# ethanhe42/epipolar-transformers

Hardware: NVIDIA B200
Metric: epipolar_fusion_forward_views_per_sec (higher is better)
Workload: dtype f32

## Files before the change

### epipolar_transformers_b200/csrc/epi_kernels.cuh

```cuda
#pragma once
#include <cuda_bf16.h>

#include "epi_common.cuh"

namespace epi {

struct FusionArgs {
    const float *feat_ref;  int64_t ref_stride[4];
    const float *src_nhwc;
    const __nv_bfloat16 *src_hi, *src_lo;
    const __nv_bfloat16 *ref_hi, *ref_lo;
    const uint16_t *order;
    const float *P_ref, *P_src;
    const float *locs_in;
    float *out;             int64_t out_stride[4];
    __nv_bfloat16 *out_hi, *out_lo;
    float *attn, *corr_pos, *locs_out;
    int N, C;
    float softmax_scale;
    int add_ref;
    int *tile_counter;
    const PairGeom *pair_geom;
    int *err_flag;
    uint8_t *plan_cache;
    int plan_records;
    const uint32_t *pair_epoch;
    GeomCfg geom;
};

struct BwdArgs {
    const float *feat_ref;  int64_t ref_stride[4];
    const float *src_nhwc;
    const float *P_ref, *P_src, *locs_in;
    const float *attn;
    const float *grad_out;  int64_t gout_stride[4];
    const float *grad_attn;
    float *grad_ref;        int64_t gref_stride[4];
    float *dsrc_nhwc;
    int N, C;
    float softmax_scale;
    int grad_keys, grad_vals;
    GeomCfg geom;
};
cudaError_t launch_fusion_bwd(const BwdArgs &a, cudaStream_t st);

struct ZArgs {
    const float *x;         int64_t x_stride[4];
    const float *ref;       int64_t ref_stride[4];
    float *y;               int64_t y_stride[4];
    const float *Wf, *bf;
    int N, C, HW, W;
    int z_residual, add_ref;
};

struct ZGemmArgs {
    const __nv_bfloat16 *x_hi, *x_lo;
    const __nv_bfloat16 *w_hi, *w_lo;
    const float *Wf, *bf;
    const float *ref;       int64_t ref_stride[4];
    float *y;               int64_t y_stride[4];
    int N, C, HW, W, Npad;
    int z_residual, add_ref;
};
bool zgemm_supported(int C);
cudaError_t launch_zgemm(const ZGemmArgs &z, cudaStream_t st);

cudaError_t launch_fusion_warp(const FusionArgs &a, cudaStream_t st);
cudaError_t launch_fusion_tile(const FusionArgs &a, cudaStream_t st);
cudaError_t launch_fusion_pipe(const FusionArgs &a, cudaStream_t st);
bool fusion_pipe_shape_ok(int C, int H, int W, int K, bool has_locs_in);
size_t fusion_pipe_plan_record_bytes();
int fusion_pipe_plan_records(int N, int H, int W);
bool fusion_tile_supported(const FusionArgs &a);
bool fusion_tile_shape_ok(int C, int H, int W, int K, bool has_locs_in);
cudaError_t launch_sector_order(const float *P_ref, const float *P_src, uint16_t *order, int N, const GeomCfg &gc, cudaStream_t st);
cudaError_t launch_split_planes(const float *src, const int64_t stride[4], __nv_bfloat16 *hi, __nv_bfloat16 *lo, int N, int C,
                                int H, int W, int *zero_me, cudaStream_t st);

cudaError_t launch_stage(const float *ref, const int64_t ref_stride[4], const float *src, const int64_t src_stride[4],
                         __nv_bfloat16 *planes, const float *P_ref, const float *P_src, PairGeom *pair_geom, uint16_t *order,
                         float *order_key, const float *Wf, __nv_bfloat16 *w_planes, int w_add_identity, int *zero_words, int N, int C,
                         int H, int W, const GeomCfg &gc, cudaStream_t st);

cudaError_t launch_nchw_to_nhwc(const float *src, const int64_t stride[4], float *dst, int N, int C, int H, int W, cudaStream_t st);
cudaError_t launch_z_epilogue(const ZArgs &z, cudaStream_t st);
cudaError_t launch_unstage(const float *pm, const float *ref, const int64_t ref_stride[4], float *out, const int64_t out_stride[4],
                           int N, int C, int H, int W, cudaStream_t st);
cudaError_t launch_fold_z_bn(const float *zw, const float *zb, const float *g, const float *b, const float *mean,
                             const float *var, float eps, int C, float *wf, float *bf, cudaStream_t st);
cudaError_t launch_peaks(const float *heat, float *locs, float *scores, int B, int J, int H, int W, float radius, float downsample,
                         float threshold, int int_div, cudaStream_t st);
cudaError_t launch_sample_locs(const float *P_ref, const float *P_src, float *locs, int N, const GeomCfg &gc, cudaStream_t st);

}
```

### epipolar_transformers_b200/csrc/epi_stage.cu

```cuda
#include <cuda_bf16.h>

#include "epi_kernels.cuh"

namespace epi {

namespace stg {
constexpr int NT = 256;
constexpr int NBIN = 4096;
constexpr int SMALL = 32;
constexpr int TC = 64, TPX = 64, TPITCH = 65;

__device__ __forceinline__ float pseudo_angle(float u, float v) {
    const float p = __fdividef(v, fabsf(u) + fabsf(v) + 1e-30f);
    return u >= 0.f ? p : (v >= 0.f ? 2.f - p : -2.f - p);
}
__device__ __forceinline__ float angle_key(float px, float py, float ex, float ey, float cdx, float cdy, bool parallel, float lo, float inv_span) {
    float u;
    if (parallel) u = (px * (-cdy) + py * cdx - lo) * inv_span;
    else {
        const float dx = px - ex, dy = py - ey;
        u = (pseudo_angle(dx * cdx + dy * cdy, dy * cdx - dx * cdy) - lo) * inv_span;
    }
    u = fminf(fmaxf(u, 0.f), 0.99999f);
    if (!(u == u)) u = 0.f;
    return u;
}
}

#ifdef EPI_PIPE_TIMERS
__device__ unsigned long long g_stage_timers[16];
#define ST(slot) do { __syncthreads(); if (t == 0 && blockIdx.x == 0) { const long long t_ = clock64(); g_stage_timers[slot] = (unsigned long long)(t_ - st_prev); st_prev = t_; } } while (0)
extern "C" void epi_stage_timers_read(unsigned long long *out16) { cudaMemcpyFromSymbol(out16, g_stage_timers, sizeof(unsigned long long) * 16); }
#else
#define ST(slot) do { } while (0)
#endif

struct StageArgs {
    const float *ref, *src;
    int64_t ref_stride[4], src_stride[4];
    __nv_bfloat16 *planes;
    const float *P_ref, *P_src;
    PairGeom *pair_geom;
    uint16_t *order;
    int *zero_words;
    float *order_key;
    const float *Wf;
    int w_add_identity;
    __nv_bfloat16 *w_planes;
    int N, C, H, W;
    int do_ref, do_src, do_order;
    int persist;
    GeomCfg gc;
};

__global__ void __launch_bounds__(stg::NT, 5) epi_stage_kernel(const StageArgs s) {
    using namespace stg;
    extern __shared__ __align__(16) uint8_t dyn[];
    float (*tile)[TPITCH] = reinterpret_cast<float (*)[TPITCH]>(dyn);
    const int t = threadIdx.x;
    const int H = s.H, W = s.W, HW = H * W, C = s.C;
    const int nord = s.do_order ? s.N : 0;
    pdl_launch_dependents();
    pdl_wait();
    if (blockIdx.x == 0 && t == 0 && s.zero_words) { s.zero_words[0] = 0; s.zero_words[1] = 0; }

    if ((int)blockIdx.x < nord) {
        int *hist = reinterpret_cast<int *>(dyn);
        uint16_t *lst = reinterpret_cast<uint16_t *>(dyn + NBIN * 4);
        __shared__ float s_e[8];
        __shared__ int s_warp[NT / 32];
        __shared__ int s_big[64], s_nbig;
#ifdef EPI_PIPE_TIMERS
        long long st_prev = clock64();
#endif
        const int n = blockIdx.x;
        float my_key = 0.f;
        if (t < 32) {
            if (t < 12) my_key = s.P_ref[12 * n + t];
            else if (t < 24) my_key = s.P_src[12 * n + t - 12];
            else if (t == 24) my_key = (float)H;
            else if (t == 25) my_key = (float)W;
            else if (t == 26) my_key = s.gc.ds;
            else if (t == 27) my_key = s.gc.r;
            else if (t == 28) my_key = 1.f;
            else if (t == 29) my_key = (float)(s.gc.K + 1024 * s.gc.correct + 2048 * s.gc.align);
            else if (t == 30) my_key = s.gc.eps;
            if (s.order_key) {
                const bool same = t == 31 || __float_as_uint(s.order_key[32 * n + t]) == __float_as_uint(my_key);
                if (__all_sync(0xffffffffu, same)) s_e[7] = 1.f; else s_e[7] = 0.f;
            } else s_e[7] = 0.f;
        }
        __syncthreads();
        if (s_e[7] != 0.f) return;
        if (t == 0) {
            const float *P1 = s.P_ref + 12 * n, *P2 = s.P_src + 12 * n;
            PairGeom g;
            pair_geom_from_krt(P1, P2, g);
            s.pair_geom[n] = g;
            double b[9], t2[3];
            for (int r = 0; r < 3; r++) { for (int q = 0; q < 3; q++) b[r * 3 + q] = (double)P2[r * 4 + q]; t2[r] = (double)P2[r * 4 + 3]; }
            const double c00 = b[4] * b[8] - b[5] * b[7], c01 = b[5] * b[6] - b[3] * b[8], c02 = b[3] * b[7] - b[4] * b[6];
            const double id = 1.0 / (b[0] * c00 + b[1] * c01 + b[2] * c02);
            double bi[9];
            bi[0] = c00 * id; bi[1] = (b[2] * b[7] - b[1] * b[8]) * id; bi[2] = (b[1] * b[5] - b[2] * b[4]) * id;
            bi[3] = c01 * id; bi[4] = (b[0] * b[8] - b[2] * b[6]) * id; bi[5] = (b[2] * b[3] - b[0] * b[5]) * id;
            bi[6] = c02 * id; bi[7] = (b[1] * b[6] - b[0] * b[7]) * id; bi[8] = (b[0] * b[4] - b[1] * b[3]) * id;
            double cs[3], e[3];
            for (int r = 0; r < 3; r++) cs[r] = -(bi[r * 3] * t2[0] + bi[r * 3 + 1] * t2[1] + bi[r * 3 + 2] * t2[2]);
            for (int r = 0; r < 3; r++) e[r] = (double)P1[r * 4] * cs[0] + (double)P1[r * 4 + 1] * cs[1] + (double)P1[r * 4 + 2] * cs[2] + (double)P1[r * 4 + 3];
            const double cx = 0.5 * ((double)s.gc.xmin + s.gc.xmax), cy = 0.5 * ((double)s.gc.ymin + s.gc.ymax);
            const double nrm = fabs(e[0]) + fabs(e[1]) + 1e-300;
            const float cxs[4] = {s.gc.xmin, s.gc.xmax, s.gc.xmin, s.gc.xmax}, cys[4] = {s.gc.ymin, s.gc.ymin, s.gc.ymax, s.gc.ymax};
            float lo = 1e30f, hi = -1e30f, exf = 0.f, eyf = 0.f, cdx, cdy, par;
            if (!(fabs(e[2]) > 1e-9 * nrm)) {
                cdx = (float)(e[0] / nrm); cdy = (float)(e[1] / nrm); par = 1.f;
                for (int q = 0; q < 4; q++) { const float v = cxs[q] * (-cdy) + cys[q] * cdx; lo = fminf(lo, v); hi = fmaxf(hi, v); }
            } else {
                const double ex = e[0] / e[2], ey = e[1] / e[2];
                const double dn = sqrt((cx - ex) * (cx - ex) + (cy - ey) * (cy - ey)) + 1e-300;
                exf = (float)ex; eyf = (float)ey; cdx = (float)((cx - ex) / dn); cdy = (float)((cy - ey) / dn); par = 0.f;
                const bool inside = ex >= s.gc.xmin && ex <= s.gc.xmax && ey >= s.gc.ymin && ey <= s.gc.ymax;
                if (inside) { lo = -2.f; hi = 2.f; }
                else
                    for (int q = 0; q < 4; q++) {
                        const float dx = cxs[q] - exf, dy = cys[q] - eyf;
                        const float v = pseudo_angle(dx * cdx + dy * cdy, dy * cdx - dx * cdy);
                        lo = fminf(lo, v); hi = fmaxf(hi, v);
                    }
            }
            if (!(hi > lo)) { lo = 0.f; hi = 1.f; }
            s_e[0] = exf; s_e[1] = eyf; s_e[2] = cdx; s_e[3] = cdy; s_e[4] = par; s_e[5] = lo; s_e[6] = 1.f / ((hi - lo) * 1.0001f + 1e-20f);
            s_nbig = 0;
        }
        for (int b = t; b < NBIN; b += NT) hist[b] = 0;
        __syncthreads();
        ST(0);
        const float ex = s_e[0], ey = s_e[1], cdx = s_e[2], cdy = s_e[3], klo = s_e[5], kinv = s_e[6];
        const bool parallel = s_e[4] != 0.f;
        constexpr int MAXPT = 64;
        const int npt = (HW - t + NT - 1) / NT;
        const bool keep = npt <= MAXPT;
        uint16_t bins[MAXPT];
        auto bin_of = [&](int x, int y) -> int {
            return (int)(angle_key(pix2coord(x, s.gc.ds, s.gc.r), pix2coord(y, s.gc.ds, s.gc.r), ex, ey, cdx, cdy, parallel, klo, kinv) * (float)NBIN);
        };
        const int sx = NT % W, sy = NT / W;
        if (keep) {
            int x = t % W, y = t / W;
#pragma unroll 4
            for (int m = 0; m < MAXPT; m++) {
                if (m < npt) {
                    const int b = bin_of(x, y);
                    bins[m] = (uint16_t)b;
                    atomicAdd(&hist[b], 1);
                    x += sx; y += sy;
                    if (x >= W) { x -= W; y++; }
                }
            }
        } else {
            int x = t % W, y = t / W;
            for (int m = 0; m < npt; m++) {
                atomicAdd(&hist[bin_of(x, y)], 1);
                x += sx; y += sy;
                if (x >= W) { x -= W; y++; }
            }
        }
        __syncthreads();
        ST(1);
        constexpr int PER = NBIN / NT;
        int loc[PER], sum = 0;
#pragma unroll
        for (int q = 0; q < PER; q++) { loc[q] = hist[t * PER + q]; sum += loc[q]; }
        int incl = sum;
#pragma unroll
        for (int o = 1; o < 32; o <<= 1) { const int v = __shfl_up_sync(0xffffffffu, incl, o); if ((t & 31) >= o) incl += v; }
        if ((t & 31) == 31) s_warp[t >> 5] = incl;
        __syncthreads();
        int base = incl - sum;
        for (int w = 0; w < (t >> 5); w++) base += s_warp[w];
        const int start0 = base;
        __syncthreads();
#pragma unroll
        for (int q = 0; q < PER; q++) { hist[t * PER + q] = base; base += loc[q]; }
        __syncthreads();
        ST(2);
        if (keep) {
#pragma unroll 4
            for (int m = 0; m < MAXPT; m++)
                if (m < npt) lst[atomicAdd(&hist[bins[m]], 1)] = (uint16_t)(t + NT * m);
        } else {
            int x = t % W, y = t / W;
            for (int m = 0; m < npt; m++) {
                lst[atomicAdd(&hist[bin_of(x, y)], 1)] = (uint16_t)(t + NT * m);
                x += sx; y += sy;
                if (x >= W) { x -= W; y++; }
            }
        }
        __syncthreads();
        ST(3);
        uint16_t *ord = s.order + (size_t)n * HW;
        {
            int st0 = start0;
#pragma unroll
            for (int q = 0; q < PER; q++) {
                const int len = loc[q];
                bool coop = false;
                if (len > (keep ? SMALL : 4 * SMALL)) {
                    const int slot = atomicAdd(&s_nbig, 1);
                    if (slot < 64) { s_big[slot] = t * PER + q; coop = true; }
                }
                if (!coop) {
                    for (int e = 1; e < len; e++) {
                        const uint16_t xv = lst[st0 + e];
                        int p = e;
                        while (p > 0 && lst[st0 + p - 1] > xv) { lst[st0 + p] = lst[st0 + p - 1]; p--; }
                        lst[st0 + p] = xv;
                    }
                }
                st0 += len;
            }
        }
        __syncthreads();
        ST(4);
        const int nbig = s_nbig < 64 ? s_nbig : 64;
        for (int i = t; i < HW; i += NT) ord[i] = lst[i];
        for (int bb = 0; bb < nbig; bb++) {
            const int b = s_big[bb];
            const int end = hist[b], beg = b == 0 ? 0 : hist[b - 1];
            __syncthreads();
            for (int e = beg + t; e < end; e += NT) {
                const uint16_t xv = lst[e];
                int r = 0;
                for (int f = beg; f < end; f++) r += lst[f] < xv;
                ord[beg + r] = xv;
            }
        }
        if (s.order_key) {
            __syncthreads();
            if (t < 31) s.order_key[32 * n + t] = my_key;
            else if (t == 31) reinterpret_cast<uint32_t *>(s.order_key)[32 * n + 31] += 1u;
        }
        return;
    }

    const int tiles_p = (HW + TPX - 1) / TPX, tiles_c = (C + TC - 1) / TC;
    const int per_map = tiles_p * tiles_c * s.N;
    int lin = (int)blockIdx.x - nord;
    const int wblocks = (s.Wf && s.w_planes) ? (C * C / 8 + NT - 1) / NT : 0;
    const int wlin = s.persist ? lin : lin - 2 * per_map;
    if (wlin >= 0 && wlin < wblocks) {
        const size_t e0 = ((size_t)wlin * NT + t) * 8, tot = (size_t)C * C;
        if (e0 < tot) {
            const float4 a4 = __ldg(reinterpret_cast<const float4 *>(s.Wf + e0)), b4 = __ldg(reinterpret_cast<const float4 *>(s.Wf + e0 + 4));
            float f[8] = {a4.x, a4.y, a4.z, a4.w, b4.x, b4.y, b4.z, b4.w};
            if (s.w_add_identity) {
                const int o = (int)(e0 / C), c_first = (int)(e0 % C);
                if (o >= c_first && o < c_first + 8) f[o - c_first] += 1.f;
            }
            uint32_t h[4], l[4];
#pragma unroll
            for (int u = 0; u < 4; u++) {
                const __nv_bfloat162 hv = __floats2bfloat162_rn(f[2 * u], f[2 * u + 1]);
                const float2 hf = __bfloat1622float2(hv);
                const __nv_bfloat162 lv = __floats2bfloat162_rn(f[2 * u] - hf.x, f[2 * u + 1] - hf.y);
                h[u] = *reinterpret_cast<const uint32_t *>(&hv);
                l[u] = *reinterpret_cast<const uint32_t *>(&lv);
            }
            *reinterpret_cast<uint4 *>(s.w_planes + e0) = make_uint4(h[0], h[1], h[2], h[3]);
            *reinterpret_cast<uint4 *>(s.w_planes + tot + e0) = make_uint4(l[0], l[1], l[2], l[3]);
        }
        return;
    }
    constexpr int QW = TPX / 4, RPP = NT / QW, RPASS = TC / RPP;
    uint32_t *whi = reinterpret_cast<uint32_t *>(dyn), *wlo = whi + TPX * 32;
    const int fq = t & 15, hsel = (t >> 4) & 1, fw = t >> 5;
    auto fast_load = [&](const float *spn, int64_t scn, int c0n, int p0n, float4 *v) {
#pragma unroll
        for (int i = 0; i < RPASS; i++) v[i] = __ldcs(reinterpret_cast<const float4 *>(spn + (int64_t)(c0n + 2 * fw + hsel + i * RPP) * scn + p0n + fq * 4));
    };
    auto fast_split = [&](const float4 *v) {
#pragma unroll
        for (int i = 0; i < RPASS; i++) {
            const float sx = hsel ? v[i].x : v[i].z, sy = hsel ? v[i].y : v[i].w;
            const float rx = __shfl_xor_sync(0xffffffffu, sx, 16), ry = __shfl_xor_sync(0xffffffffu, sy, 16);
            const float e0 = hsel ? rx : v[i].x, o0 = hsel ? v[i].z : rx;
            const float e1 = hsel ? ry : v[i].y, o1 = hsel ? v[i].w : ry;
            const int cpair = fw + 8 * i, g = cpair >> 2, k = cpair & 3;
#pragma unroll
            for (int u = 0; u < 2; u++) {
                const float fe = u ? e1 : e0, fo = u ? o1 : o0;
                const __nv_bfloat162 hv = __floats2bfloat162_rn(fe, fo);
                const float2 hf = __bfloat1622float2(hv);
                const __nv_bfloat162 lv = __floats2bfloat162_rn(fe - hf.x, fo - hf.y);
                const int px = 4 * fq + 2 * hsel + u, sw5 = (px >> 1) & 31;
                const int pos = px * 32 + (((g ^ (sw5 >> 2)) << 2) | (k ^ (sw5 & 3)));
                whi[pos] = *reinterpret_cast<const uint32_t *>(&hv);
                wlo[pos] = *reinterpret_cast<const uint32_t *>(&lv);
            }
        }
    };
    auto fast_store = [&](__nv_bfloat16 *hin, __nv_bfloat16 *lon, int nn, int c0n, int p0n) {
        const int g = t & 7, pl = t >> 3;
#pragma unroll
        for (int i = 0; i < TPX / (NT / 8); i++) {
            const int px = pl + i * (NT / 8), sw5 = (px >> 1) & 31;
            const int pos = px * 32 + ((g ^ (sw5 >> 2)) << 2);
            uint4 h4 = *reinterpret_cast<const uint4 *>(whi + pos), l4 = *reinterpret_cast<const uint4 *>(wlo + pos);
            if (sw5 & 1) { uint32_t x_; x_ = h4.x; h4.x = h4.y; h4.y = x_; x_ = h4.z; h4.z = h4.w; h4.w = x_; x_ = l4.x; l4.x = l4.y; l4.y = x_; x_ = l4.z; l4.z = l4.w; l4.w = x_; }
            if (sw5 & 2) { uint32_t x_; x_ = h4.x; h4.x = h4.z; h4.z = x_; x_ = h4.y; h4.y = h4.w; h4.w = x_; x_ = l4.x; l4.x = l4.z; l4.z = x_; x_ = l4.y; l4.y = l4.w; l4.w = x_; }
            const size_t o = ((size_t)nn * HW + p0n + px) * C + c0n + g * 8;
            *reinterpret_cast<uint4 *>(hin + o) = h4;
            *reinterpret_cast<uint4 *>(lon + o) = l4;
        }
    };
    const size_t plane_elems_all = (size_t)s.N * HW * C;
    if (s.persist) {
        const int nt = 2 * per_map, stride = s.persist;
        int cur = lin - wblocks;
        if (cur >= nt) return;
        auto decode = [&](int l, int &mp, int &nn, int &c0n, int &p0n) {
            mp = l & 1; l >>= 1;
            nn = l / (tiles_p * tiles_c);
            const int rem = l - nn * (tiles_p * tiles_c);
            const int ct = rem / tiles_p;
            c0n = ct * TC; p0n = (rem - ct * tiles_p) * TPX;
        };
        float4 v[RPASS];
        int mp, nn, c0n, p0n;
        decode(cur, mp, nn, c0n, p0n);
        fast_load((mp ? s.src : s.ref) + (int64_t)nn * (mp ? s.src_stride[0] : s.ref_stride[0]), mp ? s.src_stride[1] : s.ref_stride[1], c0n, p0n, v);
        while (true) {
            fast_split(v);
            __syncthreads();
            const int nxt = cur + stride;
            int mp2 = 0, nn2 = 0, c02 = 0, p02 = 0;
            if (nxt < nt) {
                decode(nxt, mp2, nn2, c02, p02);
                fast_load((mp2 ? s.src : s.ref) + (int64_t)nn2 * (mp2 ? s.src_stride[0] : s.ref_stride[0]), mp2 ? s.src_stride[1] : s.ref_stride[1], c02, p02, v);
            }
            __nv_bfloat16 *hin = s.planes + (size_t)(2 * mp) * plane_elems_all;
            fast_store(hin, hin + plane_elems_all, nn, c0n, p0n);
            if (nxt >= nt) return;
            __syncthreads();
            cur = nxt; mp = mp2; nn = nn2; c0n = c02; p0n = p02;
        }
    }
    int map = 0;
    if (s.do_ref && s.do_src) { map = lin & 1; lin >>= 1; }
    else map = s.do_src ? 1 : 0;
    const int n = lin / (tiles_p * tiles_c), rem = lin % (tiles_p * tiles_c);
    const int c0 = (rem / tiles_p) * TC, p0 = (rem % tiles_p) * TPX;
    const float *base = map ? s.src : s.ref;
    const int64_t *strd = map ? s.src_stride : s.ref_stride;
    const int64_t sn = strd[0], sc = strd[1], sh = strd[2], sw = strd[3];
    const float *sp = base + (int64_t)n * sn;
    const size_t plane_elems = (size_t)s.N * HW * C;
    __nv_bfloat16 *hi = s.planes + (size_t)(2 * map) * plane_elems, *lo = hi + plane_elems;
    const bool vec = (sw == 1) && (sh == W) && (HW % 4 == 0) && (sc % 4 == 0) && ((reinterpret_cast<uintptr_t>(sp) & 15) == 0);
    if (vec && sc != 1 && p0 + TPX <= HW && c0 + TC <= C) {
        float4 v[RPASS];
        fast_load(sp, sc, c0, p0, v);
        fast_split(v);
        __syncthreads();
        fast_store(hi, lo, n, c0, p0);
        return;
    }
    if (sc != 1) {
        const int q = t % QW, cy = t / QW;
        float4 v[RPASS];
#pragma unroll
        for (int i = 0; i < RPASS; i++) {
            const int c = c0 + cy + i * RPP, p = p0 + q * 4;
            v[i] = make_float4(0.f, 0.f, 0.f, 0.f);
            if (c < C) {
                if (vec && p + 3 < HW) v[i] = __ldg(reinterpret_cast<const float4 *>(sp + c * sc + p));
                else {
                    float e[4] = {0.f, 0.f, 0.f, 0.f};
                    for (int j = 0; j < 4; j++) if (p + j < HW) e[j] = __ldg(sp + c * sc + ((p + j) / W) * sh + ((p + j) % W) * sw);
                    v[i] = make_float4(e[0], e[1], e[2], e[3]);
                }
            }
        }
#pragma unroll
        for (int i = 0; i < RPASS; i++) {
            float *row = &tile[cy + i * RPP][q * 4];
            row[0] = v[i].x; row[1] = v[i].y; row[2] = v[i].z; row[3] = v[i].w;
        }
    } else {
        const int cx = t % TC, py = t / TC;
        constexpr int PPP = NT / TC;
#pragma unroll
        for (int i = 0; i < TPX / PPP; i++) {
            const int p = p0 + py + i * PPP, c = c0 + cx;
            tile[cx][py + i * PPP] = (c < C && p < HW) ? __ldg(sp + c + (p / W) * sh + (p % W) * sw) : 0.f;
        }
    }
    __syncthreads();
    constexpr int CG = TC / 8, PXP = NT / CG;
    const int cg = t % CG, pl = t / CG;
#pragma unroll
    for (int i = 0; i < TPX / PXP; i++) {
        const int pp = pl + i * PXP, p = p0 + pp, c = c0 + cg * 8;
        if (p < HW && c < C) {
            uint32_t h[4], l[4];
#pragma unroll
            for (int u = 0; u < 4; u++) {
                const float f0 = tile[cg * 8 + 2 * u][pp], f1 = tile[cg * 8 + 2 * u + 1][pp];
                const __nv_bfloat162 hv = __floats2bfloat162_rn(f0, f1);
                const float2 hf = __bfloat1622float2(hv);
                const __nv_bfloat162 lv = __floats2bfloat162_rn(f0 - hf.x, f1 - hf.y);
                h[u] = *reinterpret_cast<const uint32_t *>(&hv);
                l[u] = *reinterpret_cast<const uint32_t *>(&lv);
            }
            const size_t o = ((size_t)n * HW + p) * C + c;
            *reinterpret_cast<uint4 *>(hi + o) = make_uint4(h[0], h[1], h[2], h[3]);
            *reinterpret_cast<uint4 *>(lo + o) = make_uint4(l[0], l[1], l[2], l[3]);
        }
    }
}

cudaError_t launch_stage(const float *ref, const int64_t ref_stride[4], const float *src, const int64_t src_stride[4],
                         __nv_bfloat16 *planes, const float *P_ref, const float *P_src, PairGeom *pair_geom, uint16_t *order,
                         float *order_key, const float *Wf, __nv_bfloat16 *w_planes, int w_add_identity, int *zero_words, int N, int C,
                         int H, int W, const GeomCfg &gc, cudaStream_t st) {
    StageArgs s;
    s.ref = ref; s.src = src;
    for (int i = 0; i < 4; i++) { s.ref_stride[i] = ref_stride[i]; s.src_stride[i] = src_stride[i]; }
    s.planes = planes; s.P_ref = P_ref; s.P_src = P_src; s.pair_geom = pair_geom; s.order = order; s.order_key = order_key; s.Wf = Wf; s.w_planes = w_planes; s.w_add_identity = w_add_identity;
    s.zero_words = zero_words; s.N = N; s.C = C; s.H = H; s.W = W; s.gc = gc;
    s.do_ref = 1; s.do_src = 1; s.do_order = (P_ref && P_src && order) ? 1 : 0; s.persist = 0;
    const int tiles = ((H * W + stg::TPX - 1) / stg::TPX) * ((C + stg::TC - 1) / stg::TC) * N;
    const int wblocks = (Wf && w_planes) ? (C * C / 8 + stg::NT - 1) / stg::NT : 0;
    const size_t smem_tile = (size_t)stg::TC * stg::TPITCH * sizeof(float);
    const size_t smem_order = (size_t)stg::NBIN * 4 + (size_t)H * W * 2;
    static thread_local size_t smem_set = 0;
    auto ensure = [&](size_t smem) -> cudaError_t {
        if (smem + 1024 > 48 * 1024 && smem > smem_set) {
            cudaError_t e = cudaFuncSetAttribute(epi_stage_kernel, cudaFuncAttributeMaxDynamicSharedMemorySize, (int)smem);
            if (e != cudaSuccess) return e;
            smem_set = smem;
        }
        return cudaSuccess;
    };
    if (s.do_order && smem_order > 64 * 1024) {
        StageArgs o = s;
        o.do_ref = 0; o.do_src = 0; o.Wf = nullptr; o.w_planes = nullptr; o.persist = 0;
        cudaError_t e = ensure(smem_order);
        if (e != cudaSuccess) return e;
        e = launch_pdl(epi_stage_kernel, dim3((unsigned)N), dim3(stg::NT), smem_order, st, o);
        if (e != cudaSuccess) return e;
        s.do_order = 0; s.zero_words = nullptr;
    }
    auto whole = [&](const float *b, const int64_t *sd) {
        return sd[3] == 1 && sd[2] == W && sd[1] % 4 == 0 && sd[0] % 4 == 0 && sd[1] != 1 && (reinterpret_cast<uintptr_t>(b) & 15) == 0;
    };
    static thread_local int sms_cached = 0;
    if (!sms_cached) {
        int dev = 0;
        cudaGetDevice(&dev);
        if (cudaDeviceGetAttribute(&sms_cached, cudaDevAttrMultiProcessorCount, dev) != cudaSuccess || sms_cached <= 0) sms_cached = 148;
    }
    s.persist = 0;
    if ((H * W) % stg::TPX == 0 && C % stg::TC == 0 && whole(ref, ref_stride) && whole(src, src_stride)) {
        const int slots = 5 * sms_cached;
        s.persist = 2 * tiles < slots ? 2 * tiles : slots;
    }
    const int grid = (s.do_order ? N : 0) + wblocks + (s.persist ? s.persist : 2 * tiles);
    const size_t smem = (s.do_order && smem_order > smem_tile) ? smem_order : smem_tile;
    cudaError_t e = ensure(smem);
    if (e != cudaSuccess) return e;
    return launch_pdl(epi_stage_kernel, dim3((unsigned)grid), dim3(stg::NT), smem, st, s);
}

}
```

### epipolar_transformers_b200/csrc/epi_zgemm.cu

```cuda
#include <cuda.h>
#include <cuda_bf16.h>

#include <cstring>

#include "epi_kernels.cuh"
#include "epi_umma.cuh"

namespace epi {
using namespace umma;

namespace zg {
constexpr int NT = 256;
constexpr uint32_t A_PLANE = 16384;
constexpr int NB = 128;
constexpr uint32_t B_PLANE = 16384;
constexpr uint32_t STAGE = 2 * A_PLANE + 2 * B_PLANE;
constexpr int OT = 132;
constexpr uint32_t TILE_BYTES = NB * OT * 4;
constexpr uint32_t BUF_BYTES = TILE_BYTES > STAGE ? TILE_BYTES : STAGE;
constexpr uint32_t SMEM_ALLOC = BUF_BYTES + 1024 + 128;

__device__ __forceinline__ void tma_load_2d(void *smem_dst, const CUtensorMap *tmap, int c0, int c1, uint64_t *bar) {
    asm volatile("cp.async.bulk.tensor.2d.shared::cluster.global.mbarrier::complete_tx::bytes [%0], [%1, {%2, %3}], [%4];" ::"r"(
                     umma::smem_u32(smem_dst)),
                 "l"(tmap), "r"(c0), "r"(c1), "r"(umma::smem_u32(bar))
                 : "memory");
}
}

__global__ void __launch_bounds__(zg::NT, 2) epi_zgemm_kernel(const ZGemmArgs z, const __grid_constant__ CUtensorMap tm_hi,
                                                              const __grid_constant__ CUtensorMap tm_lo,
                                                              const __grid_constant__ CUtensorMap tw_hi,
                                                              const __grid_constant__ CUtensorMap tw_lo) {
    using namespace zg;
    extern __shared__ uint8_t smem_raw[];
    uint8_t *smem = smem_raw + ((1024u - (smem_u32(smem_raw) & 1023u)) & 1023u);
    uint64_t *bars = reinterpret_cast<uint64_t *>(smem + BUF_BYTES);
    uint32_t *tmem_slot = reinterpret_cast<uint32_t *>(smem + BUF_BYTES + 64);
    const int tid = threadIdx.x, lane = tid & 31, warp = tid >> 5;
    const int C = z.C, HW = z.HW, W = z.W;
    const int tiles = (HW + 127) / 128;
    const int n = blockIdx.x / tiles, p0 = (blockIdx.x % tiles) * 128;
    const int nq = (C + 63) / 64;
    const int oc0 = (int)blockIdx.y * NB;
    const int CO = min(NB, C - oc0);

    pdl_launch_dependents();
    const bool addr = z.ref && z.add_ref;
    const bool vec = (z.y_stride[3] == 1) && (z.y_stride[2] == W) && (HW % 4 == 0) && (z.y_stride[1] % 4 == 0) && (z.y_stride[0] % 4 == 0) &&
                     ((reinterpret_cast<uintptr_t>(z.y) & 15) == 0) &&
                     (!addr || ((z.ref_stride[3] == 1) && (z.ref_stride[2] == W) && (z.ref_stride[1] % 4 == 0) && (z.ref_stride[0] % 4 == 0) &&
                                ((reinterpret_cast<uintptr_t>(z.ref) & 15) == 0)));
    constexpr int ROWS = NB / (NT / 32);
    float4 res[ROWS];
    float bias[ROWS];
    {
        const int p = p0 + lane * 4;
#pragma unroll
        for (int k = 0; k < ROWS; k++) {
            const int ol = warp + k * (NT / 32);
            res[k] = make_float4(0.f, 0.f, 0.f, 0.f);
            bias[k] = ol < CO ? __ldg(z.bf + oc0 + ol) : 0.f;
            if (addr && vec && p + 3 < HW && ol < CO)
                res[k] = __ldcs(reinterpret_cast<const float4 *>(z.ref + (int64_t)n * z.ref_stride[0] + (int64_t)(oc0 + ol) * z.ref_stride[1] + p));
        }
    }
    if (warp == 0) tmem_alloc(tmem_slot, NB);
    if (tid == 32) { for (int i = 0; i < 3; i++) mbar_init(&bars[i], 1); mbar_fence_init(); }
    if (tid == 64) {
        asm volatile("prefetch.tensormap [%0];" ::"l"(&tm_hi) : "memory");
        asm volatile("prefetch.tensormap [%0];" ::"l"(&tm_lo) : "memory");
        asm volatile("prefetch.tensormap [%0];" ::"l"(&tw_hi) : "memory");
        asm volatile("prefetch.tensormap [%0];" ::"l"(&tw_lo) : "memory");
    }
    tc_fence_before();
    __syncthreads();
    tc_fence_after();
    const uint32_t tmem = *tmem_slot;
    pdl_wait();

    if (tid == 0) {
        const uint32_t wrows = (uint32_t)(C < NB ? C : NB);
        const uint32_t idesc = make_idesc_bf16(128, (uint32_t)((CO + 15) & ~15), 0, 0);
        for (int q = 0; q < nq; q++) {
            if (q > 0) for (uint32_t it = 0; !mbar_try_wait(&bars[1], (q - 1) & 1); ++it) if (it > (1u << 24)) __trap();
            mbar_arrive_expect_tx(&bars[0], 2 * A_PLANE + 2 * wrows * 128u);
            tma_load_2d(smem, &tm_hi, q * 64, n * HW + p0, &bars[0]);
            tma_load_2d(smem + A_PLANE, &tm_lo, q * 64, n * HW + p0, &bars[0]);
            tma_load_2d(smem + 2 * A_PLANE, &tw_hi, q * 64, oc0, &bars[0]);
            tma_load_2d(smem + 2 * A_PLANE + B_PLANE, &tw_lo, q * 64, oc0, &bars[0]);
            for (uint32_t it = 0; !mbar_try_wait(&bars[0], q & 1); ++it) if (it > (1u << 24)) __trap();
            tc_fence_after();
            const uint32_t sa = smem_u32(smem), sb = sa + 2 * A_PLANE;
#pragma unroll
            for (int ks = 0; ks < 4; ks++) {
                const uint64_t a_hi = make_smem_desc(sa + ks * 32, 16, 1024), a_lo = make_smem_desc(sa + A_PLANE + ks * 32, 16, 1024);
                const uint64_t b_hi = make_smem_desc(sb + ks * 32, 16, 1024), b_lo = make_smem_desc(sb + B_PLANE + ks * 32, 16, 1024);
                mma_bf16(tmem, a_hi, b_hi, idesc, (q | ks) ? 1u : 0u);
                mma_bf16(tmem, a_hi, b_lo, idesc, 1u);
                mma_bf16(tmem, a_lo, b_hi, idesc, 1u);
            }
            mma_commit(&bars[1]);
        }
        mma_commit(&bars[2]);
    }
    for (uint32_t it = 0; !mbar_try_wait(&bars[2], 0); ++it) if (it > (1u << 24)) __trap();
    tc_fence_after();

    float *otile = reinterpret_cast<float *>(smem);
    {
        const int r = (warp & 3) * 32 + lane;
        for (int cb = (warp >> 2) * 32; cb < CO; cb += (NT / 128) * 32) {
            float v[32];
            tmem_ld_32x32(tmem + ((uint32_t)((warp & 3) * 32) << 16) + cb, v);
            tmem_ld_wait();
#pragma unroll
            for (int jj = 0; jj < 32; jj++)
                if (cb + jj < CO) otile[(cb + jj) * OT + r] = v[jj];
        }
    }
    tc_fence_before();
    __syncthreads();
    {
        const int pp = lane * 4, p = p0 + pp;
#pragma unroll
        for (int k = 0; k < ROWS; k++) {
            const int ol = warp + k * (NT / 32);
            if (ol >= CO) break;
            const int o = oc0 + ol;
            const float4 t = *reinterpret_cast<const float4 *>(otile + ol * OT + pp);
            const float b = bias[k];
            float y[4] = {t.x + b, t.y + b, t.z + b, t.w + b};
            if (vec && p + 3 < HW) {
                __stcs(reinterpret_cast<float4 *>(z.y + (int64_t)n * z.y_stride[0] + (int64_t)o * z.y_stride[1] + p),
                       make_float4(y[0] + res[k].x, y[1] + res[k].y, y[2] + res[k].z, y[3] + res[k].w));
            } else {
                for (int e = 0; e < 4 && p + e < HW; e++) {
                    const int py = (p + e) / W, px = (p + e) % W;
                    float val = y[e];
                    if (addr) val += __ldg(z.ref + (int64_t)n * z.ref_stride[0] + (int64_t)o * z.ref_stride[1] + (int64_t)py * z.ref_stride[2] + (int64_t)px * z.ref_stride[3]);
                    z.y[(int64_t)n * z.y_stride[0] + (int64_t)o * z.y_stride[1] + (int64_t)py * z.y_stride[2] + (int64_t)px * z.y_stride[3]] = val;
                }
            }
        }
    }
    tc_fence_before();
    __syncthreads();
    if (warp == 0) tmem_dealloc(tmem, NB);
}


#ifdef EPI_PIPE_TIMERS
__device__ long long g_zg_trace[64];
__device__ unsigned long long g_zg_span[4];
#define ZTR(i) do { if (blockIdx.x == 0) g_zg_trace[i] = clock64(); } while (0)
__device__ __forceinline__ unsigned long long gtime() { unsigned long long t; asm volatile("mov.u64 %0, %globaltimer;" : "=l"(t)); return t; }
#else
#define ZTR(i) do { } while (0)
#endif
namespace zp {
constexpr int NT = 320;
constexpr int NB = 128;
constexpr int HB = 64;
constexpr int OT = 132;
constexpr uint32_t A_PLANE = 16384, A_STAGE = 2 * A_PLANE;
constexpr uint32_t W_PLANE = 16384, W_PANEL = 2 * W_PLANE;
constexpr uint32_t OFF_W = 0;
constexpr uint32_t OFF_A = 4 * W_PANEL;
constexpr uint32_t OFF_T = OFF_A + 2 * A_STAGE;
constexpr uint32_t OFF_BAR = OFF_T + HB * OT * 4;
constexpr uint32_t SMEM_ALLOC = OFF_BAR + 256 + 1024;
static_assert(SMEM_ALLOC <= 232448, "fits the opt-in shared memory");
__device__ __forceinline__ void wait_bar(uint64_t *bar, uint32_t parity) {
    for (uint32_t it = 0; !mbar_try_wait(bar, parity); ++it) if (it > (1u << 24)) __trap();
}
}

__global__ void __launch_bounds__(zp::NT, 1) epi_zgemm_persist_kernel(const ZGemmArgs z, const __grid_constant__ CUtensorMap tm_hi,
                                                                      const __grid_constant__ CUtensorMap tm_lo,
                                                                      const __grid_constant__ CUtensorMap tw_hi,
                                                                      const __grid_constant__ CUtensorMap tw_lo) {
    using namespace zp;
    extern __shared__ uint8_t smem_raw[];
    uint8_t *smem = smem_raw + ((1024u - (smem_u32(smem_raw) & 1023u)) & 1023u);
    uint64_t *bars = reinterpret_cast<uint64_t *>(smem + OFF_BAR);
    uint32_t *tmem_slot = reinterpret_cast<uint32_t *>(smem + OFF_BAR + 128);
    const int tid = threadIdx.x, lane = tid & 31, warp = tid >> 5;
    const int C = z.C, HW = z.HW, W = z.W;
    const int tiles = (HW + 127) / 128, PT = z.N * tiles;
    const int nq = (C + 63) / 64;
    const int nblk = (C + NB - 1) / NB;
    const int nb = (int)blockIdx.x % nblk, first = (int)blockIdx.x / nblk, step = (int)gridDim.x / nblk;
    const int oc0 = nb * NB, CO = min(NB, C - oc0);
#ifdef EPI_PIPE_TIMERS
    if (tid == 0) { const unsigned long long g = gtime(); atomicMin(&g_zg_span[0], g); atomicMax(&g_zg_span[1], g); }
    if (tid == 0) ZTR(0);
#endif

    pdl_launch_dependents();
    const int ew = warp - 2;
    float bias[2][HB / 8];
    if (ew >= 0) {
#pragma unroll
        for (int h = 0; h < 2; h++)
#pragma unroll
            for (int k = 0; k < HB / 8; k++) {
                const int ol = h * HB + ew + 8 * k;
                bias[h][k] = ol < CO ? __ldg(z.bf + oc0 + ol) : 0.f;
            }
    }
    if (warp == 2) tmem_alloc(tmem_slot, 256);
    if (tid == 0) {
        for (int i = 0; i < 12; i++) mbar_init(&bars[i], 1);
        mbar_fence_init();
        asm volatile("prefetch.tensormap [%0];" ::"l"(&tm_hi) : "memory");
        asm volatile("prefetch.tensormap [%0];" ::"l"(&tm_lo) : "memory");
        asm volatile("prefetch.tensormap [%0];" ::"l"(&tw_hi) : "memory");
        asm volatile("prefetch.tensormap [%0];" ::"l"(&tw_lo) : "memory");
    }
    tc_fence_before();
    __syncthreads();
    tc_fence_after();
    const uint32_t tmem = *tmem_slot;
    if (tid == 0) ZTR(1);
    pdl_wait();
    if (tid == 0) ZTR(2);

    if (warp == 0) {
        if (lane == 0 && first < PT) {
            const uint32_t wrows = (uint32_t)(C < NB ? C : NB);
            uint32_t ac = 0;
            bool first_unit = true;
            for (int pt = first; pt < PT; pt += step) {
                const int n = pt / tiles, p0 = (pt % tiles) * 128;
                for (int q = 0; q < nq; q++, ac++) {
                    if (first_unit) {
                        mbar_arrive_expect_tx(&bars[q], 2u * wrows * 128u);
                        zg::tma_load_2d(smem + OFF_W + q * W_PANEL, &tw_hi, q * 64, oc0, &bars[q]);
                        zg::tma_load_2d(smem + OFF_W + q * W_PANEL + W_PLANE, &tw_lo, q * 64, oc0, &bars[q]);
                    }
                    const uint32_t s = ac & 1u;
                    if (ac >= 2) wait_bar(&bars[6 + s], ((ac >> 1) - 1u) & 1u);
                    mbar_arrive_expect_tx(&bars[4 + s], 2 * A_PLANE);
                    zg::tma_load_2d(smem + OFF_A + s * A_STAGE, &tm_hi, q * 64, n * HW + p0, &bars[4 + s]);
                    zg::tma_load_2d(smem + OFF_A + s * A_STAGE + A_PLANE, &tm_lo, q * 64, n * HW + p0, &bars[4 + s]);
                }
                first_unit = false;
            }
        }
    } else if (warp == 1) {
        if (lane == 0 && first < PT) {
            const uint32_t idesc = make_idesc_bf16(128, (uint32_t)((CO + 15) & ~15), 0, 0);
            ZTR(3);
            uint32_t ac = 0;
            int k = 0;
            for (int pt = first; pt < PT; pt += step, k++) {
                const uint32_t buf = (uint32_t)k & 1u;
                if (k >= 2) wait_bar(&bars[10 + buf], (uint32_t)((k >> 1) - 1) & 1u);
                tc_fence_after();
                for (int q = 0; q < nq; q++, ac++) {
                    const uint32_t s = ac & 1u;
                    if (k == 0) wait_bar(&bars[q], 0);
                    wait_bar(&bars[4 + s], (ac >> 1) & 1u);
                    tc_fence_after();
                    const uint32_t sa = smem_u32(smem + OFF_A + s * A_STAGE), sb = smem_u32(smem + OFF_W + q * W_PANEL);
#pragma unroll
                    for (int ks = 0; ks < 4; ks++) {
                        const uint64_t a_hi = make_smem_desc(sa + ks * 32, 16, 1024), a_lo = make_smem_desc(sa + A_PLANE + ks * 32, 16, 1024);
                        const uint64_t b_hi = make_smem_desc(sb + ks * 32, 16, 1024), b_lo = make_smem_desc(sb + W_PLANE + ks * 32, 16, 1024);
                        mma_bf16(tmem + buf * NB, a_hi, b_hi, idesc, (q | ks) ? 1u : 0u);
                        mma_bf16(tmem + buf * NB, a_hi, b_lo, idesc, 1u);
                        mma_bf16(tmem + buf * NB, a_lo, b_hi, idesc, 1u);
                    }
                    mma_commit(&bars[6 + s]);
                }
                mma_commit(&bars[8 + buf]);
                if (k < 8) ZTR(8 + k);
            }
        }
    } else {
        float *otile = reinterpret_cast<float *>(smem + OFF_T);
        const bool addr = z.ref && z.add_ref;
        const bool vec = (z.y_stride[3] == 1) && (z.y_stride[2] == W) && (HW % 4 == 0) && (z.y_stride[1] % 4 == 0) && (z.y_stride[0] % 4 == 0) &&
                         ((reinterpret_cast<uintptr_t>(z.y) & 15) == 0) &&
                         (!addr || ((z.ref_stride[3] == 1) && (z.ref_stride[2] == W) && (z.ref_stride[1] % 4 == 0) && (z.ref_stride[0] % 4 == 0) &&
                                    ((reinterpret_cast<uintptr_t>(z.ref) & 15) == 0)));
        const int et = tid - 64;
        int k = 0;
        for (int pt = first; pt < PT; pt += step, k++) {
            const int n = pt / tiles, p0 = (pt % tiles) * 128;
            const uint32_t buf = (uint32_t)k & 1u;
            if (ew == 0) wait_bar(&bars[8 + buf], (uint32_t)(k >> 1) & 1u);
            asm volatile("bar.sync 1, 256;" ::: "memory");
            if (et == 0 && k < 8) ZTR(16 + k);
            tc_fence_after();
            const int pp = lane * 4, p = p0 + pp;
#pragma unroll
            for (int h = 0; h < 2; h++) {
                if (h * HB < CO) {
                    float4 res[HB / 8];
#pragma unroll
                    for (int kk = 0; kk < HB / 8; kk++) {
                        const int ol = h * HB + ew + 8 * kk;
                        res[kk] = make_float4(0.f, 0.f, 0.f, 0.f);
                        if (addr && vec && p + 3 < HW && ol < CO)
                            res[kk] = __ldcs(reinterpret_cast<const float4 *>(z.ref + (int64_t)n * z.ref_stride[0] + (int64_t)(oc0 + ol) * z.ref_stride[1] + p));
                    }
                    {
                        const int r = (warp & 3) * 32 + lane, cb = (ew >> 2) * 32;
                        float v[32];
                        tmem_ld_32x32(tmem + ((uint32_t)((warp & 3) * 32) << 16) + buf * NB + h * HB + cb, v);
                        tmem_ld_wait();
#pragma unroll
                        for (int jj = 0; jj < 32; jj++) otile[(cb + jj) * OT + r] = v[jj];
                    }
                    if (h == 1 || HB >= CO) tc_fence_before();
                    asm volatile("bar.sync 1, 256;" ::: "memory");
                    if ((h == 1 || HB >= CO) && et == 0) mbar_arrive(&bars[10 + buf]);
#pragma unroll
                    for (int kk = 0; kk < HB / 8; kk++) {
                        const int hl = ew + 8 * kk, ol = h * HB + hl;
                        if (ol < CO) {
                            const int o = oc0 + ol;
                            const float4 t = *reinterpret_cast<const float4 *>(otile + hl * OT + pp);
                            const float b = bias[h][kk];
                            float y[4] = {t.x + b, t.y + b, t.z + b, t.w + b};
                            if (vec && p + 3 < HW) {
                                __stcs(reinterpret_cast<float4 *>(z.y + (int64_t)n * z.y_stride[0] + (int64_t)o * z.y_stride[1] + p),
                                       make_float4(y[0] + res[kk].x, y[1] + res[kk].y, y[2] + res[kk].z, y[3] + res[kk].w));
                            } else {
                                for (int e = 0; e < 4 && p + e < HW; e++) {
                                    const int py = (p + e) / W, px = (p + e) % W;
                                    float val = y[e];
                                    if (addr) val += __ldg(z.ref + (int64_t)n * z.ref_stride[0] + (int64_t)o * z.ref_stride[1] + (int64_t)py * z.ref_stride[2] + (int64_t)px * z.ref_stride[3]);
                                    z.y[(int64_t)n * z.y_stride[0] + (int64_t)o * z.y_stride[1] + (int64_t)py * z.y_stride[2] + (int64_t)px * z.y_stride[3]] = val;
                                }
                            }
                        }
                    }
                    asm volatile("bar.sync 1, 256;" ::: "memory");
                }
            }
            if (et == 0 && k < 8) ZTR(24 + k);
        }
    }
    tc_fence_before();
    __syncthreads();
    if (warp == 2) tmem_dealloc(tmem, 256);
#ifdef EPI_PIPE_TIMERS
    if (tid == 0) { ZTR(4); const unsigned long long g = gtime(); atomicMin(&g_zg_span[2], g); atomicMax(&g_zg_span[3], g); }
#endif
}

#ifdef EPI_PIPE_TIMERS
extern "C" void epi_zgemm_trace_read(long long *out64, unsigned long long *span4, int reset) {
    cudaMemcpyFromSymbol(out64, g_zg_trace, sizeof(long long) * 64);
    cudaMemcpyFromSymbol(span4, g_zg_span, sizeof(unsigned long long) * 4);
    if (reset) { unsigned long long z4[4] = {~0ull, 0ull, ~0ull, 0ull}; cudaMemcpyToSymbol(g_zg_span, z4, sizeof(z4)); }
}
#endif

bool zgemm_supported(int C) { return C % 64 == 0 && C >= 64 && C <= 512; }

namespace {
typedef CUresult (*EncodeTiledFn)(CUtensorMap *, CUtensorMapDataType, cuuint32_t, void *, const cuuint64_t *, const cuuint64_t *,
                                  const cuuint32_t *, const cuuint32_t *, CUtensorMapInterleave, CUtensorMapSwizzle,
                                  CUtensorMapL2promotion, CUtensorMapFloatOOBfill);
EncodeTiledFn encode_fn() {
    static EncodeTiledFn fn = [] {
        void *p = nullptr;
        cudaDriverEntryPointQueryResult qr;
        if (cudaGetDriverEntryPoint("cuTensorMapEncodeTiled", &p, cudaEnableDefault, &qr) != cudaSuccess || qr != cudaDriverEntryPointSuccess) p = nullptr;
        return reinterpret_cast<EncodeTiledFn>(p);
    }();
    return fn;
}
bool make_plane_map(CUtensorMap *m, const __nv_bfloat16 *base, int rows, int C, int box_rows) {
    EncodeTiledFn fn = encode_fn();
    if (!fn || C % 8 != 0) return false;
    const cuuint64_t dims[2] = {(cuuint64_t)C, (cuuint64_t)rows};
    const cuuint64_t strides[1] = {(cuuint64_t)C * 2};
    const cuuint32_t box[2] = {64u, (cuuint32_t)box_rows};
    const cuuint32_t estr[2] = {1u, 1u};
    return fn(m, CU_TENSOR_MAP_DATA_TYPE_BFLOAT16, 2, const_cast<__nv_bfloat16 *>(base), dims, strides, box, estr,
              CU_TENSOR_MAP_INTERLEAVE_NONE, CU_TENSOR_MAP_SWIZZLE_128B, CU_TENSOR_MAP_L2_PROMOTION_L2_128B,
              CU_TENSOR_MAP_FLOAT_OOB_FILL_NONE) == CUDA_SUCCESS;
}
}

cudaError_t launch_zgemm(const ZGemmArgs &z, cudaStream_t st) {
    const int tiles = (z.HW + 127) / 128;
    const bool persist = z.C <= 256;
    static thread_local bool attr_set[2] = {false, false};
    if (!attr_set[persist ? 1 : 0]) {
        cudaError_t e = persist ? cudaFuncSetAttribute(epi_zgemm_persist_kernel, cudaFuncAttributeMaxDynamicSharedMemorySize, (int)zp::SMEM_ALLOC)
                                : cudaFuncSetAttribute(epi_zgemm_kernel, cudaFuncAttributeMaxDynamicSharedMemorySize, (int)zg::SMEM_ALLOC);
        if (e != cudaSuccess) return e;
        attr_set[persist ? 1 : 0] = true;
    }
    struct MapCache { const void *xh, *wh; int rows, C; CUtensorMap m[4]; };
    static thread_local MapCache mc = {nullptr, nullptr, 0, 0, {}};
    if (mc.xh != z.x_hi || mc.wh != z.w_hi || mc.rows != z.N * z.HW || mc.C != z.C) {
        const int wrows = z.C < zg::NB ? z.C : zg::NB;
        if (!make_plane_map(&mc.m[0], z.x_hi, z.N * z.HW, z.C, 128) || !make_plane_map(&mc.m[1], z.x_lo, z.N * z.HW, z.C, 128) ||
            !make_plane_map(&mc.m[2], z.w_hi, z.C, z.C, wrows) || !make_plane_map(&mc.m[3], z.w_lo, z.C, z.C, wrows))
            return cudaErrorInvalidValue;
        mc.xh = z.x_hi; mc.wh = z.w_hi; mc.rows = z.N * z.HW; mc.C = z.C;
    }
    if (persist) {
        static thread_local int sms_cached = 0;
        if (!sms_cached) {
            int dev = 0;
            cudaGetDevice(&dev);
            if (cudaDeviceGetAttribute(&sms_cached, cudaDevAttrMultiProcessorCount, dev) != cudaSuccess || sms_cached <= 0) sms_cached = 148;
        }
        const int nblk = (z.C + zp::NB - 1) / zp::NB, PT = z.N * tiles;
        int per = sms_cached / nblk;
        if (per > PT) per = PT;
        if (per < 1) per = 1;
        return launch_pdl(epi_zgemm_persist_kernel, dim3((unsigned)(per * nblk)), dim3(zp::NT), (size_t)zp::SMEM_ALLOC, st, z, mc.m[0], mc.m[1], mc.m[2], mc.m[3]);
    }
    return launch_pdl(epi_zgemm_kernel, dim3((unsigned)(z.N * tiles), (unsigned)((z.C + zg::NB - 1) / zg::NB)), dim3(zg::NT), (size_t)zg::SMEM_ALLOC, st, z, mc.m[0], mc.m[1], mc.m[2], mc.m[3]);
}

}
```

Before: 47150.

## Stage NCHW-to-bf16 split planes through TMA load/store ring

```diff
diff --git a/epipolar_transformers_b200/csrc/epi_kernels.cuh b/epipolar_transformers_b200/csrc/epi_kernels.cuh
--- a/epipolar_transformers_b200/csrc/epi_kernels.cuh
+++ b/epipolar_transformers_b200/csrc/epi_kernels.cuh
@@ -1,4 +1,5 @@
 #pragma once
+#include <cuda.h>
 #include <cuda_bf16.h>
 
 #include "epi_common.cuh"
@@ -63,6 +64,10 @@
     int z_residual, add_ref;
 };
 bool zgemm_supported(int C);
+typedef CUresult (*EncodeTiledFn)(CUtensorMap *, CUtensorMapDataType, cuuint32_t, void *, const cuuint64_t *, const cuuint64_t *,
+                                  const cuuint32_t *, const cuuint32_t *, CUtensorMapInterleave, CUtensorMapSwizzle,
+                                  CUtensorMapL2promotion, CUtensorMapFloatOOBfill);
+EncodeTiledFn tensor_map_encoder();
 cudaError_t launch_zgemm(const ZGemmArgs &z, cudaStream_t st);
 
 cudaError_t launch_fusion_warp(const FusionArgs &a, cudaStream_t st);
diff --git a/epipolar_transformers_b200/csrc/epi_stage.cu b/epipolar_transformers_b200/csrc/epi_stage.cu
--- a/epipolar_transformers_b200/csrc/epi_stage.cu
+++ b/epipolar_transformers_b200/csrc/epi_stage.cu
@@ -1,6 +1,9 @@
 #include <cuda_bf16.h>
 
+#include <cstring>
+
 #include "epi_kernels.cuh"
+#include "epi_umma.cuh"
 
 namespace epi {
 
@@ -9,6 +12,22 @@
 constexpr int NBIN = 4096;
 constexpr int SMALL = 32;
 constexpr int TC = 64, TPX = 64, TPITCH = 65;
+constexpr int RING = 2, TMA_PER_SM = 3;
+constexpr uint32_t TIN_BYTES = TC * TPX * 4, TOUT_BYTES = TPX * TC * 2;
+constexpr uint32_t TMA_SMEM = RING * TIN_BYTES + 4 * TOUT_BYTES + 64 + 1024;
+
+__device__ __forceinline__ uint64_t policy_evict_first() {
+    uint64_t p;
+    asm volatile("createpolicy.fractional.L2::evict_first.b64 %0, 1.0;" : "=l"(p));
+    return p;
+}
+__device__ __forceinline__ void tma_load_3d(void *dst, const CUtensorMap *tm, int px, int ch, int n, uint64_t *bar, uint64_t pol) {
+    asm volatile("cp.async.bulk.tensor.3d.shared::cluster.global.mbarrier::complete_tx::bytes.L2::cache_hint [%0], [%1, {%2, %3, %4}], [%5], %6;"
+                 ::"r"(umma::smem_u32(dst)), "l"(tm), "r"(px), "r"(ch), "r"(n), "r"(umma::smem_u32(bar)), "l"(pol) : "memory");
+}
+__device__ __forceinline__ void tma_store_2d(const CUtensorMap *tm, const void *src, int ch, int row) {
+    asm volatile("cp.async.bulk.tensor.2d.global.shared::cta.bulk_group [%0, {%1, %2}], [%3];" ::"l"(tm), "r"(ch), "r"(row), "r"(umma::smem_u32(src)) : "memory");
+}
 
 __device__ __forceinline__ float pseudo_angle(float u, float v) {
     const float p = __fdividef(v, fabsf(u) + fabsf(v) + 1e-30f);
@@ -50,10 +69,13 @@
     int N, C, H, W;
     int do_ref, do_src, do_order;
     int persist;
+    int tma;
     GeomCfg gc;
 };
 
-__global__ void __launch_bounds__(stg::NT, 5) epi_stage_kernel(const StageArgs s) {
+__global__ void __launch_bounds__(stg::NT, 5) epi_stage_kernel(const StageArgs s, const __grid_constant__ CUtensorMap tm_ref,
+                                                                const __grid_constant__ CUtensorMap tm_src,
+                                                                const __grid_constant__ CUtensorMap tm_planes) {
     using namespace stg;
     extern __shared__ __align__(16) uint8_t dyn[];
     float (*tile)[TPITCH] = reinterpret_cast<float (*)[TPITCH]>(dyn);
@@ -314,6 +336,76 @@
         }
     };
     const size_t plane_elems_all = (size_t)s.N * HW * C;
+    if (s.tma) {
+        const int nt = 2 * per_map, stride = s.persist, first = lin - wblocks;
+        if (first >= nt) return;
+        uint8_t *sm = dyn + ((1024u - (umma::smem_u32(dyn) & 1023u)) & 1023u);
+        uint8_t *sout = sm + RING * TIN_BYTES;
+        uint64_t *full = reinterpret_cast<uint64_t *>(sout + 4 * TOUT_BYTES);
+        const uint64_t pol = policy_evict_first();
+        auto decode = [&](int l, int &mp, int &nn, int &c0n, int &p0n) {
+            mp = l & 1; l >>= 1;
+            nn = l / (tiles_p * tiles_c);
+            const int rem = l - nn * (tiles_p * tiles_c);
+            const int ct = rem / tiles_p;
+            c0n = ct * TC; p0n = (rem - ct * tiles_p) * TPX;
+        };
+        auto issue = [&](int l, int slot) {
+            int mp, nn, c0n, p0n;
+            decode(l, mp, nn, c0n, p0n);
+            umma::mbar_arrive_expect_tx(&full[slot], TIN_BYTES);
+            tma_load_3d(sm + slot * TIN_BYTES, mp ? &tm_src : &tm_ref, p0n, c0n, nn, &full[slot], pol);
+        };
+        if (t == 0) {
+            asm volatile("prefetch.tensormap [%0];" ::"l"(&tm_ref) : "memory");
+            asm volatile("prefetch.tensormap [%0];" ::"l"(&tm_src) : "memory");
+            asm volatile("prefetch.tensormap [%0];" ::"l"(&tm_planes) : "memory");
+            for (int r = 0; r < RING; r++) umma::mbar_init(&full[r], 1);
+            umma::mbar_fence_init();
+            for (int r = 0; r < RING; r++) if (first + r * stride < nt) issue(first + r * stride, r);
+        }
+        __syncthreads();
+        const int px = t & (TPX - 1), cq = t / TPX;
+        int j = 0;
+        for (int l = first; l < nt; l += stride, j++) {
+            const int slot = j % RING, ob = j & 1;
+            int mp, nn, c0n, p0n;
+            decode(l, mp, nn, c0n, p0n);
+            if (t == 0) asm volatile("cp.async.bulk.wait_group.read 1;" ::: "memory");
+            for (uint32_t it = 0; !umma::mbar_try_wait(&full[slot], (uint32_t)(j / RING) & 1u); ++it) if (it > (1u << 24)) __trap();
+            __syncthreads();
+            const float *f32 = reinterpret_cast<const float *>(sm + slot * TIN_BYTES);
+            uint8_t *oh = sout + ob * 2 * TOUT_BYTES, *ol = oh + TOUT_BYTES;
+#pragma unroll
+            for (int k = 0; k < 2; k++) {
+                const int cg = 2 * cq + k;
+                uint32_t h[4], lw[4];
+#pragma unroll
+                for (int u = 0; u < 4; u++) {
+                    const float f0 = f32[(cg * 8 + 2 * u) * TPX + px], f1 = f32[(cg * 8 + 2 * u + 1) * TPX + px];
+                    const __nv_bfloat162 hv = __floats2bfloat162_rn(f0, f1);
+                    const float2 hf = __bfloat1622float2(hv);
+                    const __nv_bfloat162 lv = __floats2bfloat162_rn(f0 - hf.x, f1 - hf.y);
+                    h[u] = *reinterpret_cast<const uint32_t *>(&hv);
+                    lw[u] = *reinterpret_cast<const uint32_t *>(&lv);
+                }
+                const int off = px * 128 + ((cg ^ (px & 7)) << 4);
+                *reinterpret_cast<uint4 *>(oh + off) = make_uint4(h[0], h[1], h[2], h[3]);
+                *reinterpret_cast<uint4 *>(ol + off) = make_uint4(lw[0], lw[1], lw[2], lw[3]);
+            }
+            umma::fence_proxy_async_smem();
+            __syncthreads();
+            if (t == 0) {
+                const int row = nn * HW + p0n;
+                tma_store_2d(&tm_planes, oh, c0n, (2 * mp) * s.N * HW + row);
+                tma_store_2d(&tm_planes, ol, c0n, (2 * mp + 1) * s.N * HW + row);
+                asm volatile("cp.async.bulk.commit_group;" ::: "memory");
+                if (l + RING * stride < nt) issue(l + RING * stride, slot);
+            }
+        }
+        if (t == 0) asm volatile("cp.async.bulk.wait_group 0;" ::: "memory");
+        return;
+    }
     if (s.persist) {
         const int nt = 2 * per_map, stride = s.persist;
         int cur = lin - wblocks;
@@ -428,7 +520,7 @@
     for (int i = 0; i < 4; i++) { s.ref_stride[i] = ref_stride[i]; s.src_stride[i] = src_stride[i]; }
     s.planes = planes; s.P_ref = P_ref; s.P_src = P_src; s.pair_geom = pair_geom; s.order = order; s.order_key = order_key; s.Wf = Wf; s.w_planes = w_planes; s.w_add_identity = w_add_identity;
     s.zero_words = zero_words; s.N = N; s.C = C; s.H = H; s.W = W; s.gc = gc;
-    s.do_ref = 1; s.do_src = 1; s.do_order = (P_ref && P_src && order) ? 1 : 0; s.persist = 0;
+    s.do_ref = 1; s.do_src = 1; s.do_order = (P_ref && P_src && order) ? 1 : 0; s.persist = 0; s.tma = 0;
     const int tiles = ((H * W + stg::TPX - 1) / stg::TPX) * ((C + stg::TC - 1) / stg::TC) * N;
     const int wblocks = (Wf && w_planes) ? (C * C / 8 + stg::NT - 1) / stg::NT : 0;
     const size_t smem_tile = (size_t)stg::TC * stg::TPITCH * sizeof(float);
@@ -447,7 +539,8 @@
         o.do_ref = 0; o.do_src = 0; o.Wf = nullptr; o.w_planes = nullptr; o.persist = 0;
         cudaError_t e = ensure(smem_order);
         if (e != cudaSuccess) return e;
-        e = launch_pdl(epi_stage_kernel, dim3((unsigned)N), dim3(stg::NT), smem_order, st, o);
+        const CUtensorMap none = {};
+        e = launch_pdl(epi_stage_kernel, dim3((unsigned)N), dim3(stg::NT), smem_order, st, o, none, none, none);
         if (e != cudaSuccess) return e;
         s.do_order = 0; s.zero_words = nullptr;
     }
@@ -460,16 +553,52 @@
         cudaGetDevice(&dev);
         if (cudaDeviceGetAttribute(&sms_cached, cudaDevAttrMultiProcessorCount, dev) != cudaSuccess || sms_cached <= 0) sms_cached = 148;
     }
-    s.persist = 0;
+    s.persist = 0; s.tma = 0;
+    struct MapCache { const void *ref, *src, *planes; int64_t rs[4], ss[4]; int N, C, HW, dev; bool ok; CUtensorMap m[3]; };
+    static thread_local MapCache mc = {};
+    static const CUtensorMap no_map = {};
     if ((H * W) % stg::TPX == 0 && C % stg::TC == 0 && whole(ref, ref_stride) && whole(src, src_stride)) {
-        const int slots = 5 * sms_cached;
+        int dev = 0;
+        cudaGetDevice(&dev);
+        if (mc.ref != ref || mc.src != src || mc.planes != planes || memcmp(mc.rs, ref_stride, sizeof(mc.rs)) != 0 ||
+            memcmp(mc.ss, src_stride, sizeof(mc.ss)) != 0 || mc.N != N || mc.C != C || mc.HW != H * W || mc.dev != dev) {
+            mc.ref = ref; mc.src = src; mc.planes = planes; mc.N = N; mc.C = C; mc.HW = H * W; mc.dev = dev;
+            memcpy(mc.rs, ref_stride, sizeof(mc.rs)); memcpy(mc.ss, src_stride, sizeof(mc.ss));
+            auto local = [&](const void *p) {
+                cudaPointerAttributes a;
+                if (cudaPointerGetAttributes(&a, p) != cudaSuccess) { cudaGetLastError(); return false; }
+                return a.type == cudaMemoryTypeDevice && a.device == dev;
+            };
+            EncodeTiledFn enc = tensor_map_encoder();
+            auto map_in = [&](CUtensorMap *m, const float *b, const int64_t *sd) {
+                const cuuint64_t dims[3] = {(cuuint64_t)H * W, (cuuint64_t)C, (cuuint64_t)N};
+                const cuuint64_t strides[2] = {(cuuint64_t)sd[1] * 4, (cuuint64_t)sd[0] * 4};
+                const cuuint32_t box[3] = {stg::TPX, stg::TC, 1}, es[3] = {1, 1, 1};
+                return enc(m, CU_TENSOR_MAP_DATA_TYPE_FLOAT32, 3, const_cast<float *>(b), dims, strides, box, es, CU_TENSOR_MAP_INTERLEAVE_NONE,
+                           CU_TENSOR_MAP_SWIZZLE_NONE, CU_TENSOR_MAP_L2_PROMOTION_L2_256B, CU_TENSOR_MAP_FLOAT_OOB_FILL_NONE) == CUDA_SUCCESS;
+            };
+            auto map_out = [&](CUtensorMap *m) {
+                const cuuint64_t dims[2] = {(cuuint64_t)C, (cuuint64_t)4 * N * H * W};
+                const cuuint64_t strides[1] = {(cuuint64_t)C * 2};
+                const cuuint32_t box[2] = {stg::TC, stg::TPX}, es[2] = {1, 1};
+                return enc(m, CU_TENSOR_MAP_DATA_TYPE_BFLOAT16, 2, planes, dims, strides, box, es, CU_TENSOR_MAP_INTERLEAVE_NONE,
+                           CU_TENSOR_MAP_SWIZZLE_128B, CU_TENSOR_MAP_L2_PROMOTION_L2_128B, CU_TENSOR_MAP_FLOAT_OOB_FILL_NONE) == CUDA_SUCCESS;
+            };
+            mc.ok = enc && (reinterpret_cast<uintptr_t>(planes) & 15) == 0 && local(ref) && local(src) && local(planes) &&
+                    map_in(&mc.m[0], ref, ref_stride) && map_in(&mc.m[1], src, src_stride) && map_out(&mc.m[2]);
+        }
+        s.tma = mc.ok ? 1 : 0;
+        const int slots = (s.tma ? stg::TMA_PER_SM : 5) * sms_cached;
         s.persist = 2 * tiles < slots ? 2 * tiles : slots;
     }
     const int grid = (s.do_order ? N : 0) + wblocks + (s.persist ? s.persist : 2 * tiles);
-    const size_t smem = (s.do_order && smem_order > smem_tile) ? smem_order : smem_tile;
+    size_t smem = (s.do_order && smem_order > smem_tile) ? smem_order : smem_tile;
+    if (s.tma && smem < stg::TMA_SMEM) smem = stg::TMA_SMEM;
     cudaError_t e = ensure(smem);
     if (e != cudaSuccess) return e;
-    return launch_pdl(epi_stage_kernel, dim3((unsigned)grid), dim3(stg::NT), smem, st, s);
-}
-
-}
+    const CUtensorMap *tm = s.tma ? mc.m : nullptr;
+    return launch_pdl(epi_stage_kernel, dim3((unsigned)grid), dim3(stg::NT), smem, st, s, tm ? tm[0] : no_map, tm ? tm[1] : no_map,
+                      tm ? tm[2] : no_map);
+}
+
+}
diff --git a/epipolar_transformers_b200/csrc/epi_zgemm.cu b/epipolar_transformers_b200/csrc/epi_zgemm.cu
--- a/epipolar_transformers_b200/csrc/epi_zgemm.cu
+++ b/epipolar_transformers_b200/csrc/epi_zgemm.cu
@@ -362,11 +362,7 @@
 
 bool zgemm_supported(int C) { return C % 64 == 0 && C >= 64 && C <= 512; }
 
-namespace {
-typedef CUresult (*EncodeTiledFn)(CUtensorMap *, CUtensorMapDataType, cuuint32_t, void *, const cuuint64_t *, const cuuint64_t *,
-                                  const cuuint32_t *, const cuuint32_t *, CUtensorMapInterleave, CUtensorMapSwizzle,
-                                  CUtensorMapL2promotion, CUtensorMapFloatOOBfill);
-EncodeTiledFn encode_fn() {
+EncodeTiledFn tensor_map_encoder() {
     static EncodeTiledFn fn = [] {
         void *p = nullptr;
         cudaDriverEntryPointQueryResult qr;
@@ -375,8 +371,10 @@
     }();
     return fn;
 }
+
+namespace {
 bool make_plane_map(CUtensorMap *m, const __nv_bfloat16 *base, int rows, int C, int box_rows) {
-    EncodeTiledFn fn = encode_fn();
+    EncodeTiledFn fn = tensor_map_encoder();
     if (!fn || C % 8 != 0) return false;
     const cuuint64_t dims[2] = {(cuuint64_t)C, (cuuint64_t)rows};
     const cuuint64_t strides[1] = {(cuuint64_t)C * 2};
```

Measured after the change: 48510 (median of 6 runs). +2.9%, better.
